# groupeLIAMG/ttcr

Measured on AMD Instinct MI355X. Metric: Mnodes/s per sweep-iteration (512^3 fp32 grid, first-order FSM), higher is better.
Workload: dtype f32

## Files before the change

### include/ttcr_amd.h

```cpp
#ifndef TTCR_AMD_H
#define TTCR_AMD_H

#include <stddef.h>
#include <stdint.h>

#ifdef __cplusplus
extern "C" {
#endif

typedef struct ttcr_fsm_grid ttcr_fsm_grid;

enum { TTCR_F32 = 0, TTCR_F64 = 1 };

enum {
    TTCR_OK = 0,
    TTCR_ERR_VALUE = 1,
    TTCR_ERR_RUNTIME = 2,
    TTCR_ERR_DEVICE = 3,
    TTCR_ERR_UNSUPPORTED = 4
};

int ttcr_fsm_device_count(void);

const char* ttcr_fsm_last_error(void);
// ... 121 lines not shown
int ttcr_fsm_multi_l_size(const ttcr_fsm_grid* g, size_t* n_rows, size_t* nnz);
int ttcr_fsm_get_multi_l(const ttcr_fsm_grid* g, long long* row_off, long long* cell, void* v);

typedef struct {
    double sweep_ms;
    double total_ms;
    long long kernel_launches;
    long long node_updates;
    long long evaluated_updates;
    int iterations;
    int n_sources;
} ttcr_fsm_timing;
int ttcr_fsm_last_timing(const ttcr_fsm_grid* g, ttcr_fsm_timing* out);
int ttcr_fsm_stopping_stats(const ttcr_fsm_grid* g, long long* reference_sums, long long* reference_sums_missed, long long* rounds);
int ttcr_fsm_prefill_swaps(const ttcr_fsm_grid* g, long long* swaps);
int ttcr_fsm_reference_change(ttcr_fsm_grid* g, const void* times, const void* field, int parallel, void* out);
int ttcr_fsm_last_kernel(const ttcr_fsm_grid* g, char* buf, size_t n);
int ttcr_fsm_unit_order(int dim, int dtype, int stage, int by_time, uint32_t nnx, uint32_t nny, uint32_t nnz, uint32_t* out,
                        size_t capacity, size_t* n_units);
const char* ttcr_fsm_build_id(void);

#ifdef __cplusplus
}
#endif
#endif
```

### ttcr_amd/_lib.py

```python
import ctypes as C
import os

HERE = os.path.dirname(os.path.abspath(__file__))
LIB_PATH = os.environ.get("TTCR_AMD_LIB") or os.path.join(HERE, "libttcr_amd.so")

TTCR_F32, TTCR_F64 = 0, 1
OK, ERR_VALUE, ERR_RUNTIME, ERR_DEVICE, ERR_UNSUPPORTED = 0, 1, 2, 3, 4

_P = C.c_void_p
_U32 = C.c_uint32
_D = C.c_double
_I = C.c_int


class Timing(C.Structure):
    _fields_ = [("sweep_ms", C.c_double), ("total_ms", C.c_double), ("kernel_launches", C.c_longlong),
                ("node_updates", C.c_longlong), ("evaluated_updates", C.c_longlong), ("iterations", C.c_int),
                ("n_sources", C.c_int)]


SYMBOLS = {
    "ttcr_fsm_device_count": (_I, []),
    "ttcr_fsm_last_error": (C.c_char_p, []),
    "ttcr_fsm3d_create": (_I, [C.POINTER(_P), _I, _I, _U32, _U32, _U32, _D, _D, _D, _D, _D, _I, _I, _I, _I, _I]),
# ... 14 lines not shown
    "ttcr_fsm_interp": (_I, [_P, _I, _I, _P, _P]),
    "ttcr_fsm_compute_slowness": (_I, [_P, _I, _P, _I, _P]),
    "ttcr_fsm_get_niter": (_I, [_P, _I, C.POINTER(_I), C.POINTER(_I)]),
    "ttcr_fsm_get_changes": (_I, [_P, _I, C.POINTER(_D), _I, C.POINTER(_D), _I]),
    "ttcr_fsm_get_reference_changes": (_I, [_P, _I, C.POINTER(_D), _I, C.POINTER(_D), _I]),
    "ttcr_fsm_n_slots": (_I, [_P]),
    "ttcr_fsm_n_nodes": (C.c_size_t, [_P]),
    "ttcr_fsm_n_cells": (C.c_size_t, [_P]),
    "ttcr_fsm_set_option": (_I, [_P, C.c_char_p, _D]),
    "ttcr_fsm_last_timing": (_I, [_P, C.POINTER(Timing)]),
    "ttcr_fsm_last_kernel": (_I, [_P, C.c_char_p, C.c_size_t]),
    "ttcr_fsm_build_id": (C.c_char_p, []),
    "ttcr_fsm_unit_order": (_I, [_I, _I, _I, _I, _U32, _U32, _U32, C.POINTER(_U32), C.c_size_t, C.POINTER(C.c_size_t)]),
    "ttcr_fsm_stopping_stats": (_I, [_P, C.POINTER(C.c_longlong), C.POINTER(C.c_longlong), C.POINTER(C.c_longlong)]),
    "ttcr_fsm_prefill_swaps": (_I, [_P, C.POINTER(C.c_longlong)]),
    "ttcr_fsm_reference_change": (_I, [_P, C.c_void_p, C.c_void_p, C.c_int, C.c_void_p]),
    "ttcr_fsm_rays_size": (_I, [_P, C.POINTER(C.c_size_t), C.POINTER(C.c_size_t)]),
    "ttcr_fsm_get_rays": (_I, [_P, _P, _P]),
    "ttcr_fsm_raytrace_rays": (_I, [_P, _I, _I, _P, _P, _I, _P, _P]),
    "ttcr_fsm_slot_rays_size": (_I, [_P, _I, C.POINTER(C.c_size_t), C.POINTER(C.c_size_t)]),
    "ttcr_fsm_get_slot_rays": (_I, [_P, _I, _P, _P]),
    "ttcr_fsm_raytrace_m": (_I, [_P, _I, _I, _P, _P, _I, _P, _P]),
    "ttcr_fsm_raytrace_rm": (_I, [_P, _I, _I, _P, _P, _I, _P, _P]),
    "ttcr_fsm_raytrace_multi_m": (_I, [_P, _I, _P, _P, _P, _P, _P, _P, _I]),
    "ttcr_fsm_multi_m_size": (_I, [_P, C.POINTER(C.c_size_t), C.POINTER(C.c_size_t)]),
    "ttcr_fsm_get_multi_m": (_I, [_P, _P, _P, _P]),
    "ttcr_fsm_raytrace_multi_tape": (_I, [_P, _I, _P, _P, _P, _P, _P, _P, C.POINTER(_P)]),
    "ttcr_fsm_tape_size": (_I, [_P, C.POINTER(C.c_size_t), C.POINTER(C.c_size_t), C.POINTER(C.c_size_t)]),
    "ttcr_fsm_tape_bytes": (_I, [_P, C.POINTER(C.c_size_t)]),
    "ttcr_fsm_tape_device": (_I, [_P, C.POINTER(_I)]),
# ... 89 lines not shown
```

### ttcr_amd/build.py

```python
import os
import shutil
import subprocess

HERE = os.path.dirname(os.path.abspath(__file__))
CSRC = os.path.join(HERE, "csrc")
OBJ = os.path.join(CSRC, "_obj")
LIB = os.path.join(HERE, "libttcr_amd.so")
INC = os.path.join("..", "..", "include", "ttcr_amd.h")
UNITS = {
    "fsm_capi.hip": ([], ["fsm_capi.hip", "fsm_kernels.h", "fsm_fast_api.h", "fsm_march_levels.inc", "fsm_fast.hip", "fsm_tape_api.h",
                          "fsm_tape.hip", "fsm_adjoint_api.h", "fsm_adjoint.hip", "fsm_unit_order.h", INC]),
    "fsm_fast.hip": ([], ["fsm_fast.hip", "fsm_fast_api.h", "fsm_kernels.h", "fsm_march_levels.inc"]),
    "fsm_tape.hip": ([], ["fsm_tape.hip", "fsm_tape_api.h"]),
    "fsm_adjoint.hip": ([], ["fsm_adjoint.hip", "fsm_adjoint_api.h", "fsm_kernels.h", "fsm_march_levels.inc"]),
}
SOURCES = list(UNITS)
DEPS = sorted({d for _, ds in UNITS.values() for d in ds})
FLAGS = ["--offload-arch=gfx950", "-O3", "-std=c++17", "-fPIC", "-ffp-contract=off",
         "-fno-fast-math", "-Wall", "-Wno-unused-result"]


def _hipcc():
    for c in (os.environ.get("HIPCC"), shutil.which("hipcc"), "/opt/rocm/bin/hipcc"):
        if c and os.path.exists(c):
            return c
    raise RuntimeError("hipcc not found")


def source_hash():
# ... 50 lines not shown
```

### ttcr_amd/csrc/fsm_capi.hip

```cpp
#include <hip/hip_runtime.h>

#include <algorithm>
#include <atomic>
#include <chrono>
#include <condition_variable>
#include <cmath>
#include <cstdio>
#include <cstdlib>
#include <cstring>
#include <limits>
#include <map>
#include <memory>
#include <mutex>
#include <sstream>
#include <stdexcept>
#include <string>
#include <thread>
#include <vector>

#include "../../include/ttcr_amd.h"
#include "fsm_kernels.h"
#include "fsm_fast_api.h"
#include "fsm_tape_api.h"
#include "fsm_adjoint_api.h"
// ... 117 lines not shown
    std::vector<int> niter, niterw;
    std::vector<int> phys;
    int P(int slot) const { return phys.empty() ? slot : phys[slot]; }
    int stopping_shortcuts = 3;
    int stopping_rule = 1;
    long long reference_sums = 0, reference_sums_missed = 0;
    long long refsum_rounds = 0;
    virtual void stopping_stats(long long* sums, long long* missed, long long* rounds) const {
        if (sums) *sums = reference_sums;
        if (missed) *missed = reference_sums_missed;
        if (rounds) *rounds = refsum_rounds;
    }
    virtual void reference_change_host(const void* times, const void* field, bool parallel, void* out) = 0;
    int pair_by_distance = 1;
    virtual void set_pair_layout(int) {}
    virtual long long prefill_swap_count() const { return 0; }
    int lone_chunk = 16;
    int arith = 0;
    int prefill = -1;
    std::vector<std::vector<double>> change_hist, change_histw;
    std::vector<std::vector<double>> ref_hist, ref_histw;
    virtual void get_reference_changes(int slot, double* first, int n_first, double* wen, int n_weno) const {
        if (slot < 0 || slot >= n_slots) throw ValueError("Thread number is larger than number of threads");
        slot = P(slot);
        for (int q = 0; q < n_first; ++q) first[q] = (!ref_hist.empty() && q < (int)ref_hist[slot].size()) ? ref_hist[slot][q] : std::nan("");
        for (int q = 0; q < n_weno; ++q) wen[q] = (!ref_histw.empty() && q < (int)ref_histw[slot].size()) ? ref_histw[slot][q] : std::nan("");
    }
    virtual void get_changes(int slot, double* first, int n_first, double* wen, int n_weno) const {
        if (slot < 0 || slot >= n_slots) throw ValueError("Thread number is larger than number of threads");
        slot = P(slot);
        for (int q = 0; q < n_first; ++q) first[q] = (!change_hist.empty() && q < (int)change_hist[slot].size()) ? change_hist[slot][q] : 0.0;
        for (int q = 0; q < n_weno; ++q) wen[q] = (!change_histw.empty() && q < (int)change_histw[slot].size()) ? change_histw[slot][q] : 0.0;
    }
    bool weno = false;
// ... 18 lines not shown
        else if (k == "mode") mode = (int)value;
        else if (k == "skip") skip = (int)value;
        else if (k == "tt_from_rp") ttrp = value != 0;
        else if (k == "interp_vel") interp_vel = value != 0;
        else if (k == "return_rays") return_rays = value != 0;
        else if (k == "pair_sources") pair_by_distance = value != 0;
        else if (k == "pair_layout") {
            if (value != -1 && value != 0 && value != 1) throw ValueError("option 'pair_layout': -1 (default), 0 or 1");
            set_pair_layout((int)value);
        }
        else if (k == "stopping_rule") stopping_rule = (int)value;
        else if (k == "stopping_shortcuts") { if (value < 0 || value > 3 || value != (double)(int)value) throw ValueError("option stopping_shortcuts: 0 ... 3"); stopping_shortcuts = (int)value; }
        else if (k == "prefill") {
            if (value != -1 && value != 0 && value != 1) throw ValueError("option 'prefill': -1 (default), 0 or 1");
            prefill = (int)value;
        } else if (k == "lone_chunk") {
            if (value != 8 && value != 16) throw ValueError("option 'lone_chunk': 8 or 16");
            lone_chunk = (int)value;
        }
        else if (k == "arith") {
            if (value != 0 && value != 1 && value != 2)
                throw ValueError("option 'arith': 0 (the reference's arithmetic), 1 (tolerance-grade fp32 where it stays within 1e-5 s RMS) or 2 (the WENO stage as well)");
            arith = (int)value;
        }
        else if (k == "walk_records") {
            if (value != 0 && !(value >= 1 && value <= (double)walk_step_limit && value == (double)(long)value))
                throw ValueError("option 'walk_records': 0 (default) or a whole number from 1 to the step limit of a walk");
            walk_records = (long)value;
        }
        else throw ValueError("unknown option '" + k + "'");
// ... 31 lines not shown
    T dx, dz, xmin, ymin, zmin, xmax, ymax, zmax, ox = 0, oy = 0, oz = 0;
    T epsilon;
    int nitermax;
    bool cell, translate;
    bool have_slowness = false;

    hipStream_t stream = nullptr;
    hipEvent_t ev0 = nullptr, ev1 = nullptr;
    DevBuf<T> d_s, d_cells, d_tt, d_rx, d_out;
    DevBuf<T> d_tt_alt;
    bool alt_filled = false;
    hipStream_t fill_stream = nullptr;
    hipEvent_t ev_fill = nullptr;
    long long prefill_swaps = 0;
    long long prefill_swap_count() const override { return prefill_swaps; }
    void set_pair_layout(int v) override { pair_layout = v; }
    DevBuf<int> d_rslot;
    DevBuf<RaySrc> d_rdesc;
    int weno_ch4_min = 8;
    int weno_c16_below = 3;
    int f64_c16_below = 5;
    int pre_min = 2;
    size_t xs_lds_bytes = 40000;
    int xs_lds_below = 2;
    size_t xs_dyn_lds(int batch) const { return (dim == 3 && stage == 0 && batch < xs_lds_below) ? xs_lds_bytes : 0; }
    int time_order_below = 1 << 30;
    DevBuf<T> d_gather;
    DevBuf<T> d_rsrc, d_rt0;
    DevBuf<int> d_rstat;
    DevBuf<T> d_ssh;
// ... 81 lines not shown
        }
        HIP_CHECK(hipStreamCreateWithFlags(&stream, hipStreamNonBlocking));
        HIP_CHECK(hipEventCreate(&ev0));
        HIP_CHECK(hipEventCreate(&ev1));
        d_s.reserve(n_nodes, 64);
        {
            long long pair_units_min = 6144;
            if (const char* e = std::getenv("TTCR_FSM_PAIR_UNITS")) pair_units_min = std::atoll(e);
            const long long patches = dim == 3 ? (long long)((ny + 1 + TileCfg<T, 3>::PJ - 1) / TileCfg<T, 3>::PJ) * ((nz + 1 + TileCfg<T, 3>::PK - 1) / TileCfg<T, 3>::PK) : 0;
            NS = (n_slots >= 2 && dim == 3 && !weno && (long long)n_slots * patches > pair_units_min) ? 2 : 1;
            ns_window = NS == 2 && (long long)n_slots * patches <= (5 * pair_units_min) / 2;
        }
        if (const char* e = std::getenv("TTCR_FSM_PAIR")) { NS = (std::atoi(e) != 0 && n_slots >= 2) ? 2 : 1; ns_window = false; }
        if (const char* e = std::getenv("TTCR_FSM_LAYOUT_LO")) layout_lo = std::atof(e);
        if (const char* e = std::getenv("TTCR_FSM_LAYOUT_HI")) layout_hi = std::atof(e);
        d_tt.reserve(n_nodes * (size_t)(n_slots + (n_slots & 1)), 64);
        mask_words = (n_nodes + 31) / 32;
        d_mask.reserve(mask_words * (size_t)n_slots);
        d_bbox.reserve(6 * (size_t)n_slots);
        d_slots.reserve(n_slots);
        d_lmask.reserve(n_slots);
        HIP_CHECK(hipHostMalloc((void**)&h_lmask, sizeof(int) * n_slots));
        d_change.reserve(n_slots);
        if (std::getenv("TTCR_FSM_PROF")) {
            prof_words = 8 + 4 * (size_t)(1 << 20);
            d_prof.reserve(prof_words);
            HIP_CHECK(hipMemset(d_prof.p, 0, prof_words * sizeof(unsigned long long)));
        }
        HIP_CHECK(hipHostMalloc((void**)&h_change, sizeof(double) * n_slots));
        HIP_CHECK(hipHostMalloc((void**)&h_slots, sizeof(int) * n_slots));
        HIP_CHECK(hipHostMalloc((void**)&h_abort, sizeof(int)));
        *h_abort = 0;
        HIP_CHECK(hipHostMalloc((void**)&h_iter, 2 * sizeof(int)));
        HIP_CHECK(hipHostMalloc((void**)&h_evals, sizeof(unsigned long long) * n_slots));
        HIP_CHECK(hipMemsetAsync(d_tt.p, 0, n_nodes * (size_t)(n_slots + (n_slots & 1)) * sizeof(T), stream));

        if (dim == 3) {
            using C = TileCfg<T, 3>;
            geom.NF = nx + 1; geom.NJ = ny + 1; geom.NK = nz + 1;
            geom.npj = (geom.NJ + C::PJ - 1) / C::PJ;
            geom.npk = (geom.NK + C::PK - 1) / C::PK;
            n_launch = count_launches(C::BL);
        } else {
            using C = TileCfg<T, 2>;
            geom.NF = nz + 1; geom.NJ = nx + 1; geom.NK = 1;
            geom.npj = (geom.NJ + C::PJ - 1) / C::PJ;
            geom.npk = 1;
            n_launch = count_launches(C::BL);
        }
        geom.n_nodes = (uint32_t)n_nodes;
// ... 113 lines not shown
        pa.sync = d_sync.p;
        pa.n_patches = n_patches;
        pa.batch = batch;
        pa.timeout_ticks = 300000000ull;
        pa.stamp = d_stamp.p;
        pa.iter_ptr = d_iter.p;
        pa.evals = d_evals.p;
        pa.nbf = nbf; pa.nbj = nbj; pa.nbk = nbk;
        pa.ndir = DIM == 3 ? 8 : 4;
        pa.skip = skip_now(batch) ? (std::getenv("TTCR_FSM_SKIP_ALL_DIRTY") ? 2 : 1) : 0;
        pa.cmap = d_cmap.p;
        pa.cw = cmap_words;
        pa.sw = std::getenv("TTCR_FSM_NO_SW") ? nullptr : d_sw.p;
        pa.n_sw_groups = n_groups();
        pa.n_sw_sweeps = sw_sweeps;

        const size_t wg_cap = (fsm_looped(DIM == 3, H) && persist_wgs > 0) ? (size_t)persist_wgs : ~(size_t)0;
        const dim3 block(C::PJ * C::PK), grid((unsigned)std::min<size_t>((size_t)n_patches * batch, wg_cap));
        const int ndir = DIM == 3 ? 8 : 4;
        {
            const bool pre_ = mode == 2 && !NO_PRE && (DIM == 2 || batch >= pre_min || dyn_lds > 0);
            char nm[160];
            std::snprintf(nm, sizeof nm, "fsm_sweep_persistent<%s,%d,%d,%d,%s,%s,%d,%d,%s,%s>", sizeof(T) == 4 ? "float" : "double", C::PJ, C::PK, CH,
                          DIM == 3 ? "true" : "false", skip_now(batch) ? "true" : "false", H, NSV, mode == 2 ? "true" : "false", pre_ ? "true" : "false");
            last_kernel = nm;
        }
        if (mode == 2) {
            pa.ssh = d_ssh.p;
            pa.ssh_stride = ssh_stride;
            pa.dir = 0;
            a.rf = a.rj = a.rk = a.rev = 0;
            a.s_sheared = nullptr;
            pa.timeout_ticks = 1000000000ull;
            const dim3 gridx((unsigned)std::min<size_t>((size_t)n_patches * batch * ndir, wg_cap));
            pa.order = d_order_xs[H == 2 ? 1 : 0][batch < time_order_below ? 1 : 0].p;
            const bool pre = DIM == 2 || batch >= pre_min || dyn_lds > 0;
            if constexpr (std::is_same<T, float>::value) {
                if (fast_now<H>() && (H == 1 || NSV == 1)) {
                    const FastCfg fc{H, DIM, NSV, CH, skip_now(batch), NO_PRE ? false : pre};
                    last_kernel.insert(last_kernel.size() - 1, ",1");
                    const hipError_t e = fsm_fast_launch(pa, fc, gridx.x, dyn_lds, stream);
                    if (e == hipErrorInvalidValue) throw std::logic_error("arith = 1: no such kernel (" + last_kernel + ")");
                    HIP_CHECK(e);
                    return;
                }
            }
            if constexpr (NO_PRE) {
                (void)pre;
                if (skip_now(batch))
                    fsm_sweep_persistent<T, C::PJ, C::PK, CH, DIM == 3, true, H, NSV, true><<<gridx, block, dyn_lds, stream>>>(pa);
                else
// ... 305 lines not shown
    bool ns_window = false;
    int pair_layout = -1;
    double last_eval_frac = -1;
    double layout_lo = 0.55, layout_hi = 0.70;
    void choose_layout() {
        if (!ns_window) return;
        int want = NS;
        if (pair_layout >= 0) want = pair_layout ? 2 : 1;
        else if (last_eval_frac >= 0) want = NS == 2 ? (last_eval_frac < layout_lo ? 1 : 2) : (last_eval_frac > layout_hi ? 2 : 1);
        if (want == NS) return;
        NS = want;
        graph_batches[0] = graph_batches[1] = -1;
        for (int q = 0; q < n_slots; ++q) phys[q] = q;
    }
    int n_groups() const { return (n_slots + NS - 1) / NS; }
    T* tt_ptr(int slot) const { return d_tt.p + (size_t)(slot / NS) * n_nodes * NS + slot % NS; }
    template <int H>
    bool fast_now() const { return sizeof(T) == 4 && (arith == 2 || (arith == 1 && !weno)); }
    bool prefill_on() const {
        if (prefill >= 0) return prefill != 0;
        const size_t bytes = n_nodes * (size_t)(n_slots + (n_slots & 1)) * sizeof(T);
        if (bytes < ((size_t)64 << 20)) return false;
        size_t free_b = 0, total_b = 0;
        if (hipMemGetInfo(&free_b, &total_b) != hipSuccess) return false;
        return d_tt_alt.p || (2 * bytes <= total_b / 2 && bytes + ((size_t)1 << 30) <= free_b);
    }

    int stage = 0;
    int skip_units_min = 2048;
    int skip_probe_min = 1024;
    bool probe_skip = true;
    int probe_off_calls = 0;
    int persist_wgs = 2048;
    bool in_probe_window(int entries) const {
        const long long u = (long long)n_patches * entries;
        return dim == 3 && sizeof(T) == 4 && u >= skip_probe_min && u < skip_units_min;
    }
    int skip_default(int entries) const {
        if (dim != 3) return 1;
        if (stage == 1) return 1;
// ... 384 lines not shown
        size_t tot_pts = 0;
        for (int b = 0; b < nb; ++b) tot_pts += tx_off[src_ids[b] + 1] - tx_off[src_ids[b]];
        std::vector<InitPoint<T>> pts;
        pts.reserve(tot_pts);
        std::vector<size_t> first(nb);
        for (int b = 0; b < nb; ++b) {
            first[b] = pts.size();
            for (int n = tx_off[src_ids[b]]; n < tx_off[src_ids[b] + 1]; ++n) pts.push_back(locate(tx + (size_t)nc * n, t0[n]));
        }
        d_pts.reserve(std::max<size_t>(tot_pts, 1));
        HIP_CHECK(hipMemcpyAsync(d_pts.p, pts.data(), pts.size() * sizeof(InitPoint<T>), hipMemcpyHostToDevice, stream));
        for (int b = 0; b < nb; ++b)
            HIP_CHECK(hipMemsetAsync(d_stamp.p + (size_t)(slot_ids[b] / NS) * n_bricks, 0xFF, n_bricks * sizeof(int), stream));
        std::vector<char> group_filled(n_groups(), 0);
        const bool all_slots = nb == n_slots && prefill_on();
        if (all_slots && alt_filled) {
            HIP_CHECK(hipStreamWaitEvent(stream, ev_fill, 0));
            std::swap(d_tt.p, d_tt_alt.p);
            std::swap(d_tt.n, d_tt_alt.n);
            std::swap(d_tt.guard, d_tt_alt.guard);
            alt_filled = false;
            ++prefill_swaps;
            graph_batches[0] = graph_batches[1] = -1;
            std::fill(group_filled.begin(), group_filled.end(), 1);
        }
        if (NS > 1) {
            std::vector<int> cnt(n_groups(), 0);
            for (int b = 0; b < nb; ++b) cnt[slot_ids[b] / NS] += 1;
            for (int gi = 0; gi < n_groups(); ++gi) {
                if (cnt[gi] != NS || group_filled[gi]) continue;
// ... 82 lines not shown
                } else {
                    n_entries = nb;
                    for (int b = 0; b < nb; ++b) { h_slots[b] = b < (int)active.size() ? active[b] : -1; h_lmask[b] = 1; }
                }
                HIP_CHECK(hipMemcpyAsync(d_slots.p, h_slots, sizeof(int) * n_entries, hipMemcpyHostToDevice, stream));
                HIP_CHECK(hipMemcpyAsync(d_lmask.p, h_lmask, sizeof(int) * n_entries, hipMemcpyHostToDevice, stream));
                HIP_CHECK(hipMemsetAsync(d_change.p, 0, sizeof(double) * n_slots, stream));
                iter_T = it_total;
                snapshots_before_iteration(active, it + 1);
                if (host_prof) { HIP_CHECK(hipStreamSynchronize(stream)); hp_mark("snapshots"); }
                stamps_ok = (it == 0 ? true : stamps_ok) && stamps_live_for(n_entries);
                h_iter[0] = it_total;
                h_iter[1] = (int)launch_epoch;
                launch_epoch += (persistent_now() && mode == 2) ? 1u : (unsigned)ndir;
                HIP_CHECK(hipMemcpyAsync(d_iter.p, h_iter, 2 * sizeof(int), hipMemcpyHostToDevice, stream));
                run_iteration(n_entries);
                HIP_CHECK(hipMemcpyAsync(h_change, d_change.p, sizeof(double) * n_slots, hipMemcpyDeviceToHost, stream));
                if (persistent_now()) HIP_CHECK(hipMemcpyAsync(h_abort, d_sync.p + 4, sizeof(int), hipMemcpyDeviceToHost, stream));
                HIP_CHECK(hipStreamSynchronize(stream));
                hp_mark("sweep-iteration");
                if (persistent_now() && *h_abort) {
                    HIP_CHECK(hipMemsetAsync(d_sync.p + 4, 0, sizeof(int), stream));
                    stage = 0;
                    throw DeviceError("persistent sweep kernel: a patch timed out waiting for its upwind neighbour");
                }
                ++it;
                ++it_total;
                std::vector<int> next;
                if (fixed_iters > 0) ref_change_last.assign(n_slots, std::nan(""));
                const std::vector<char> go = fixed_iters > 0 ? std::vector<char>(active.size(), 1) : decide_go_on(active, it);
                hp_mark("stopping rule");
                for (size_t q = 0; q < active.size(); ++q) {
                    const int s2 = active[q];
                    (stage == 0 ? niter : niterw)[s2] = it;
                    (stage == 0 ? change_hist : change_histw)[s2].push_back(h_change[s2]);
                    (stage == 0 ? ref_hist : ref_histw)[s2].push_back((int)ref_change_last.size() == n_slots ? ref_change_last[s2] : std::nan(""));
                    timing.node_updates += (long long)n_nodes * ndir;
                    prev2_change[s2] = prev_change[s2];
                    prev_change[s2] = h_change[s2];
                    if (go[q]) next.push_back(s2);
// ... 6 lines not shown
                for (int s2 : slot_ids)
                    HIP_CHECK(hipMemsetD32Async((hipDeviceptr_t)(d_stamp.p + (size_t)(s2 / NS) * n_bricks), it_total * (dim == 3 ? 8 : 4),
                                                n_bricks, stream));
            }
        }
        if (std::getenv("TTCR_FSM_DEBUG_SW")) {
            std::vector<unsigned long long> h((size_t)std::min(sw_sweeps, 40) * n_groups());
            HIP_CHECK(hipMemcpy(h.data(), d_sw.p, h.size() * sizeof(unsigned long long), hipMemcpyDeviceToHost));
            for (size_t q = 0; q < h.size(); ++q) std::fprintf(stderr, "%s%u/%u", q % n_groups() == 0 ? "\n[sw] " : " ", (unsigned)h[q], (unsigned)(h[q] >> 32));
            std::fprintf(stderr, "\n");
        }
        const bool was_persistent = mode >= 1 || weno;
        stage = 0;
        sync_clean = true;
        HIP_CHECK(hipEventRecord(ev1, stream));
        if (all_slots) {
            const size_t n_el = n_nodes * (size_t)(n_slots + (n_slots & 1));
            if (!fill_stream) {
                int lo = 0, hi = 0;
                HIP_CHECK(hipDeviceGetStreamPriorityRange(&lo, &hi));
                HIP_CHECK(hipStreamCreateWithPriority(&fill_stream, hipStreamNonBlocking, lo));
                HIP_CHECK(hipEventCreateWithFlags(&ev_fill, hipEventDisableTiming));
            }
            bool have_alt = true;
            try {
                d_tt_alt.reserve(n_el, 64);
            } catch (const DeviceError&) {
                (void)hipGetLastError();
                have_alt = false;
                prefill = 0;
            }
            if (have_alt) {
// ... 1070 lines not shown
        for (auto& r : rep) r->apply_option(k, value);
    }
    void set_slowness(const void* s, size_t n, bool on_device, bool c_order = false) override {
        for (auto& r : rep) r->set_slowness(s, n, on_device, c_order);
    }
    void get_slowness(void* out, size_t n) override { rep[0]->get_slowness(out, n); }
    void validate_points(int n_tx, const void* tx, int n_rx, const void* rx) override { rep[0]->validate_points(n_tx, tx, n_rx, rx); }
    void get_tt(int slot, void* out, size_t n) override { int l; GridBase& g = of(slot, l); g.get_tt(l, out, n); }
    void* tt_device(int slot) override { int l; GridBase& g = of(slot, l); return g.tt_device(l); }
    void* tt_device_view(int slot, size_t* stride) override { int l; GridBase& g = of(slot, l); return g.tt_device_view(l, stride); }
    void interp(int slot, int n, const void* pts, void* out) override { int l; GridBase& g = of(slot, l); g.interp(l, n, pts, out); }
    void compute_slowness(int n, const void* pts, bool translated, void* out) override { rep[0]->compute_slowness(n, pts, translated, out); }
    void get_niter(int slot, int* it, int* itw) const override { int l; GridBase& g = of(slot, l); g.get_niter(l, it, itw); }
    std::string kernel_name() const override { return rep[0]->kernel_name(); }
    long long prefill_swap_count() const override { long long a = 0; for (const auto& r : rep) a += r->prefill_swap_count(); return a; }
    void stopping_stats(long long* sums, long long* missed, long long* rounds) const override {
        long long a = 0, b = 0, c = 0;
        for (const auto& r : rep) { long long x = 0, y = 0, z = 0; r->stopping_stats(&x, &y, &z); a += x; b += y; c += z; }
        if (sums) *sums = a;
        if (missed) *missed = b;
        if (rounds) *rounds = c;
    }
    void reference_change_host(const void* times, const void* field, bool parallel, void* out) override { rep[0]->reference_change_host(times, field, parallel, out); }
    void get_changes(int slot, double* first, int n_first, double* wen, int n_weno) const override {
        int l; GridBase& g = of(slot, l); g.get_changes(l, first, n_first, wen, n_weno);
    }
    void get_reference_changes(int slot, double* first, int n_first, double* wen, int n_weno) const override {
        int l; GridBase& g = of(slot, l); g.get_reference_changes(l, first, n_first, wen, n_weno);
    }
    void rays_size(size_t* n_rays, size_t* n_points) const override { *n_rays = rays_off.size() - 1; *n_points = (size_t)rays_off.back(); }
// ... 1247 lines not shown
        out->total_ms = t.total_ms;
        out->kernel_launches = t.launches;
        out->node_updates = t.node_updates;
        out->evaluated_updates = t.evaluated_updates;
        out->iterations = t.iterations;
        out->n_sources = t.n_sources;
    });
}

int ttcr_fsm_stopping_stats(const ttcr_fsm_grid* g, long long* reference_sums, long long* reference_sums_missed, long long* rounds) {
    return guarded_on(g, [&] { g->impl->stopping_stats(reference_sums, reference_sums_missed, rounds); });
}
int ttcr_fsm_prefill_swaps(const ttcr_fsm_grid* g, long long* swaps) {
    return guarded_on(g, [&] { if (swaps) *swaps = g->impl->prefill_swap_count(); });
}
int ttcr_fsm_reference_change(ttcr_fsm_grid* g, const void* times, const void* field, int parallel, void* out) {
    return guarded_on(g, [&] {
        if (!times || !field || !out) throw ValueError("ttcr_fsm_reference_change: null argument");
        g->impl->reference_change_host(times, field, parallel != 0, out);
    });
}

int ttcr_fsm_last_kernel(const ttcr_fsm_grid* g, char* buf, size_t n) {
    return guarded_on(g, [&] {
        if (!buf || n == 0) throw ValueError("ttcr_fsm_last_kernel: no buffer");
        const std::string k = g->impl->kernel_name();
        std::snprintf(buf, n, "%s", k.c_str());
    });
}

// ... 16 lines not shown
        } else {
            PJ = dim == 3 ? TileCfg<double, 3>::PJ : TileCfg<double, 2>::PJ; PK = dim == 3 ? TileCfg<double, 3>::PK : 1;
            C = dim == 3 ? ChunkCfg<double, 3>::C : ChunkCfg<double, 2>::C;
        }
        const uint64_t npj = ((uint64_t)NJ + PJ - 1) / PJ, npk = ((uint64_t)NK + PK - 1) / PK;
        if (NF >= (1u << 30) || npj >= (1u << 14) || npk >= (1u << 14)) throw ValueError("grid too large for the patch index of the sweep kernel");
        *n_units = (size_t)(npj * npk) * (dim == 3 ? 8 : 4);
        if (!out) return;
        if (capacity < *n_units) throw ValueError("output buffer too small for the units of the launch");
        const std::vector<uint32_t> xs = fsm_xs_order(dim, (int)NF, (int)NJ, (int)NK, PJ, PK, C, stage == 0 ? 1 : 2, by_time != 0,
                                                      fsm_diag_order((int)npj, (int)npk));
        std::copy(xs.begin(), xs.end(), out);
    });
}

const char* ttcr_fsm_build_id(void) { return TTCR_BUILD_ID; }

}
```

### ttcr_amd/csrc/fsm_kernels.h

```cpp
#pragma once
#include <hip/hip_runtime.h>
#include <stdint.h>
#include <type_traits>

namespace ttcr_amd {

constexpr int FSM_BRICK = 16;

template <typename T> struct real_traits;
template <> struct real_traits<float> {
    static __host__ __device__ constexpr float max() { return 3.402823466e+38f; }
    static __device__ __forceinline__ float inf() { return __builtin_huge_valf(); }
};
template <> struct real_traits<double> {
    static __host__ __device__ constexpr double max() { return 1.7976931348623157e+308; }
    static __device__ __forceinline__ double inf() { return __builtin_huge_val(); }
};

__device__ __forceinline__ uint32_t idx_u32(double v) { return v < 0 ? 0u : (v >= 4294967295.0 ? 4294967295u : (uint32_t)v); }

__device__ __forceinline__ float rmin(float a, float b) { return a < b ? a : b; }
__device__ __forceinline__ double rmin(double a, double b) { return a < b ? a : b; }
__device__ __forceinline__ float rmax(float a, float b) { return a < b ? b : a; }
__device__ __forceinline__ double rmax(double a, double b) { return a < b ? b : a; }
// ... 404 lines not shown
    int* sync;
    int n_patches, batch;
    unsigned long long timeout_ticks;
    int* stamp;
    const int* iter_ptr;
    unsigned long long* evals;
    int nbf, nbj, nbk;
    int dir, ndir;
    int skip;
    unsigned long long* cmap;
    int cw;
    unsigned long long* sw;
    int n_sw_groups, n_sw_sweeps;
    const T* ssh;
    size_t ssh_stride;
};



__device__ __forceinline__ float ld_sc1(const float* p) {
    return __uint_as_float(__hip_atomic_load((const unsigned int*)p, __ATOMIC_RELAXED, __HIP_MEMORY_SCOPE_AGENT));
}
__device__ __forceinline__ double ld_sc1(const double* p) {
    return __longlong_as_double(__hip_atomic_load((const long long*)p, __ATOMIC_RELAXED, __HIP_MEMORY_SCOPE_AGENT));
}
__device__ __forceinline__ void st_sc1(float* p, float v) {
    __hip_atomic_store((unsigned int*)p, __float_as_uint(v), __ATOMIC_RELAXED, __HIP_MEMORY_SCOPE_AGENT);
}
__device__ __forceinline__ void st_sc1(double* p, double v) {
    __hip_atomic_store((long long*)p, __double_as_longlong(v), __ATOMIC_RELAXED, __HIP_MEMORY_SCOPE_AGENT);
// ... 409 lines not shown
        const int tka = IS3D ? ka2 / PK : 0, ntk = IS3D ? kb2 / PK - tka + 1 : 1;
        const int ia = lane & 3, ib = lane >> 2;
        if (ia >= ntj || ib >= ntk) return nullptr;
        return pa.sync + 8 + ((size_t)pd * pa.batch + z_) * pa.n_patches + ((tka + ib) * npj + tja + ia);
    };
    if constexpr (LOOPED) __syncthreads();
    if (tid == 0) {
        const int t_ = atomicAdd(pa.sync + (epoch & 3u), 1);
        if (t_ == 0) __hip_atomic_store(pa.sync + ((epoch + 2u) & 3u), 0, __ATOMIC_RELAXED, __HIP_MEMORY_SCOPE_AGENT);
        s_ticket = t_;
    }
    if (LOOPED && tid == 1) s_abort = __hip_atomic_load(pa.sync + 4, __ATOMIC_RELAXED, __HIP_MEMORY_SCOPE_AGENT);
    __syncthreads();
    if (LOOPED && s_abort) return false;
    const int ticket = __builtin_amdgcn_readfirstlane(s_ticket);
    const int oidx = ticket / pa.batch, z = ticket - oidx * pa.batch;
    if (oidx >= (XS ? pa.n_patches * pa.ndir : pa.n_patches)) return false;
    if (FSM_ENABLE_PROF == 1 && a.prof && ticket < 8192) prec = a.prof + 8 + 4 * 65536 + (size_t)ticket * 400;
    const uint32_t tile = pa.order[oidx];
    const int dir = XS ? (int)(tile >> 28) : pa.dir;
    const int TJ = XS ? (int)(tile & 0x3fffu) : (int)(tile & 0xffffu), TK = XS ? (int)((tile >> 14) & 0x3fffu) : (int)(tile >> 16);
    int* prog = pa.sync + 8 + ((size_t)(XS ? dir : 0) * pa.batch + z) * pa.n_patches;
    int* my_prog = prog + (TK * npj + TJ);
    int rf, rj, rk, rev;
    const T* __restrict__ Sg;
    if (XS) {
        int fam;
        if (IS3D) {
            rf = dir & 1; rj = (dir >> 1) & 1; rk = (dir >> 2) & 1;
            rev = rk;
// ... 2560 lines not shown
```

### ttcr_amd/rgrid.py

```python
import ctypes as C
import math

import numpy as np

from . import _lib

_verbose = 0


def set_verbose(v):
    global _verbose
    _verbose = int(v)


def _ptr(a):
    return a.ctypes.data_as(C.c_void_p)


def _row_groups(a):
    key = np.ascontiguousarray(a, dtype=np.float64) + 0.0
    n = key.shape[0]
    if n == 0:
        return np.zeros(0, dtype=np.intp), np.zeros(1, dtype=np.intp), key
    ne = key[1:] != key[:-1]
# ... 86 lines not shown
        return np.array(a[:n1]), np.array(b[:n2])

    def timing(self):
        t = _lib.Timing()
        _lib.check(self._lib.ttcr_fsm_last_timing(self._h, C.byref(t)))
        return {k: getattr(t, k) for k, _ in t._fields_}

    def stopping_stats(self):
        a, b, c = C.c_longlong(0), C.c_longlong(0), C.c_longlong(0)
        _lib.check(self._lib.ttcr_fsm_stopping_stats(self._h, C.byref(a), C.byref(b), C.byref(c)))
        return {"reference_sums": a.value, "reference_sums_missed": b.value, "rounds": c.value}

    def prefill_swaps(self):
        a = C.c_longlong(0)
        _lib.check(self._lib.ttcr_fsm_prefill_swaps(self._h, C.byref(a)))
        return a.value

    def reference_change(self, times, field, parallel=True):
        dt = self._dtype
        a = np.ascontiguousarray(times, dtype=dt).ravel()
        b = np.ascontiguousarray(field, dtype=dt).ravel()
        n = self.get_number_of_nodes()
        if a.size != n or b.size != n:
            raise ValueError('reference_change: fields of get_number_of_nodes() values expected')
        out = np.zeros(1, dtype=dt)
        _lib.check(self._lib.ttcr_fsm_reference_change(self._h, a.ctypes.data, b.ctypes.data, 1 if parallel else 0, out.ctypes.data))
        return out[0]

    def last_kernel(self):
        buf = C.create_string_buffer(256)
# ... 1250 lines not shown
```

Baseline: 94390.

## Fuse alternate travel-time buffer prefill into first sweep iteration kernel

Instead of filling the alternate travel-time buffer with max values on a separate low-priority stream after the solve, each sweep work-group writes a vectorized slice of that buffer at the start of its ticket during the first iteration. The aim is to hide the prefill memory traffic inside the sweep launch and avoid a separate fill pass competing for bandwidth. It also trims the tt allocation to omit the odd-slot padding when pairing is off. The cost is extra stores and register pressure in the sweep kernel prologue on every ticket of that iteration, plus a per-ticket branch checked in all launches.

```diff
diff --git a/include/ttcr_amd.h b/include/ttcr_amd.h
--- a/include/ttcr_amd.h
+++ b/include/ttcr_amd.h
@@ -159,10 +159,12 @@
 int ttcr_fsm_last_timing(const ttcr_fsm_grid* g, ttcr_fsm_timing* out);
 int ttcr_fsm_stopping_stats(const ttcr_fsm_grid* g, long long* reference_sums, long long* reference_sums_missed, long long* rounds);
 int ttcr_fsm_prefill_swaps(const ttcr_fsm_grid* g, long long* swaps);
+int ttcr_fsm_prefill_inline_fills(const ttcr_fsm_grid* g, long long* fills);
 int ttcr_fsm_reference_change(ttcr_fsm_grid* g, const void* times, const void* field, int parallel, void* out);
 int ttcr_fsm_last_kernel(const ttcr_fsm_grid* g, char* buf, size_t n);
 int ttcr_fsm_unit_order(int dim, int dtype, int stage, int by_time, uint32_t nnx, uint32_t nny, uint32_t nnz, uint32_t* out,
                         size_t capacity, size_t* n_units);
+int ttcr_fsm_prefill_slice(int dtype, uint64_t n_el, uint32_t n_tickets, uint32_t ticket, uint64_t* slice_len, uint64_t* begin, uint64_t* end);
 const char* ttcr_fsm_build_id(void);
 
 #ifdef __cplusplus
diff --git a/ttcr_amd/_lib.py b/ttcr_amd/_lib.py
--- a/ttcr_amd/_lib.py
+++ b/ttcr_amd/_lib.py
@@ -52,6 +52,8 @@
     "ttcr_fsm_unit_order": (_I, [_I, _I, _I, _I, _U32, _U32, _U32, C.POINTER(_U32), C.c_size_t, C.POINTER(C.c_size_t)]),
     "ttcr_fsm_stopping_stats": (_I, [_P, C.POINTER(C.c_longlong), C.POINTER(C.c_longlong), C.POINTER(C.c_longlong)]),
     "ttcr_fsm_prefill_swaps": (_I, [_P, C.POINTER(C.c_longlong)]),
+    "ttcr_fsm_prefill_inline_fills": (_I, [_P, C.POINTER(C.c_longlong)]),
+    "ttcr_fsm_prefill_slice": (_I, [_I, C.c_uint64, _U32, _U32, C.POINTER(C.c_uint64), C.POINTER(C.c_uint64), C.POINTER(C.c_uint64)]),
     "ttcr_fsm_reference_change": (_I, [_P, C.c_void_p, C.c_void_p, C.c_int, C.c_void_p]),
     "ttcr_fsm_rays_size": (_I, [_P, C.POINTER(C.c_size_t), C.POINTER(C.c_size_t)]),
     "ttcr_fsm_get_rays": (_I, [_P, _P, _P]),
diff --git a/ttcr_amd/build.py b/ttcr_amd/build.py
--- a/ttcr_amd/build.py
+++ b/ttcr_amd/build.py
@@ -9,10 +9,10 @@
 INC = os.path.join("..", "..", "include", "ttcr_amd.h")
 UNITS = {
     "fsm_capi.hip": ([], ["fsm_capi.hip", "fsm_kernels.h", "fsm_fast_api.h", "fsm_march_levels.inc", "fsm_fast.hip", "fsm_tape_api.h",
-                          "fsm_tape.hip", "fsm_adjoint_api.h", "fsm_adjoint.hip", "fsm_unit_order.h", INC]),
-    "fsm_fast.hip": ([], ["fsm_fast.hip", "fsm_fast_api.h", "fsm_kernels.h", "fsm_march_levels.inc"]),
+                          "fsm_tape.hip", "fsm_adjoint_api.h", "fsm_adjoint.hip", "fsm_unit_order.h", "fsm_prefill_slices.h", INC]),
+    "fsm_fast.hip": ([], ["fsm_fast.hip", "fsm_fast_api.h", "fsm_kernels.h", "fsm_march_levels.inc", "fsm_prefill_slices.h"]),
     "fsm_tape.hip": ([], ["fsm_tape.hip", "fsm_tape_api.h"]),
-    "fsm_adjoint.hip": ([], ["fsm_adjoint.hip", "fsm_adjoint_api.h", "fsm_kernels.h", "fsm_march_levels.inc"]),
+    "fsm_adjoint.hip": ([], ["fsm_adjoint.hip", "fsm_adjoint_api.h", "fsm_kernels.h", "fsm_march_levels.inc", "fsm_prefill_slices.h"]),
 }
 SOURCES = list(UNITS)
 DEPS = sorted({d for _, ds in UNITS.values() for d in ds})
diff --git a/ttcr_amd/csrc/fsm_capi.hip b/ttcr_amd/csrc/fsm_capi.hip
--- a/ttcr_amd/csrc/fsm_capi.hip
+++ b/ttcr_amd/csrc/fsm_capi.hip
@@ -155,10 +155,12 @@
     virtual void reference_change_host(const void* times, const void* field, bool parallel, void* out) = 0;
     int pair_by_distance = 1;
     virtual void set_pair_layout(int) {}
+    virtual long long prefill_inline_count() const { return 0; }
     virtual long long prefill_swap_count() const { return 0; }
     int lone_chunk = 16;
     int arith = 0;
     int prefill = -1;
+    int prefill_inline = -1;
     std::vector<std::vector<double>> change_hist, change_histw;
     std::vector<std::vector<double>> ref_hist, ref_histw;
     virtual void get_reference_changes(int slot, double* first, int n_first, double* wen, int n_weno) const {
@@ -207,6 +209,9 @@
         else if (k == "prefill") {
             if (value != -1 && value != 0 && value != 1) throw ValueError("option 'prefill': -1 (default), 0 or 1");
             prefill = (int)value;
+        } else if (k == "prefill_inline") {
+            if (value != -1 && value != 0 && value != 1) throw ValueError("option 'prefill_inline': -1 (default), 0 or 1");
+            prefill_inline = (int)value;
         } else if (k == "lone_chunk") {
             if (value != 8 && value != 16) throw ValueError("option 'lone_chunk': 8 or 16");
             lone_chunk = (int)value;
@@ -268,6 +273,8 @@
     hipEvent_t ev_fill = nullptr;
     long long prefill_swaps = 0;
     long long prefill_swap_count() const override { return prefill_swaps; }
+    long long prefill_inline_fills = 0;
+    long long prefill_inline_count() const override { return prefill_inline_fills; }
     void set_pair_layout(int v) override { pair_layout = v; }
     DevBuf<int> d_rslot;
     DevBuf<RaySrc> d_rdesc;
@@ -379,7 +386,7 @@
         if (const char* e = std::getenv("TTCR_FSM_PAIR")) { NS = (std::atoi(e) != 0 && n_slots >= 2) ? 2 : 1; ns_window = false; }
         if (const char* e = std::getenv("TTCR_FSM_LAYOUT_LO")) layout_lo = std::atof(e);
         if (const char* e = std::getenv("TTCR_FSM_LAYOUT_HI")) layout_hi = std::atof(e);
-        d_tt.reserve(n_nodes * (size_t)(n_slots + (n_slots & 1)), 64);
+        d_tt.reserve(n_nodes * tt_fields(), 64);
         mask_words = (n_nodes + 31) / 32;
         d_mask.reserve(mask_words * (size_t)n_slots);
         d_bbox.reserve(6 * (size_t)n_slots);
@@ -398,7 +405,7 @@
         *h_abort = 0;
         HIP_CHECK(hipHostMalloc((void**)&h_iter, 2 * sizeof(int)));
         HIP_CHECK(hipHostMalloc((void**)&h_evals, sizeof(unsigned long long) * n_slots));
-        HIP_CHECK(hipMemsetAsync(d_tt.p, 0, n_nodes * (size_t)(n_slots + (n_slots & 1)) * sizeof(T), stream));
+        HIP_CHECK(hipMemsetAsync(d_tt.p, 0, n_nodes * tt_fields() * sizeof(T), stream));
 
         if (dim == 3) {
             using C = TileCfg<T, 3>;
@@ -542,6 +549,9 @@
         pa.sw = std::getenv("TTCR_FSM_NO_SW") ? nullptr : d_sw.p;
         pa.n_sw_groups = n_groups();
         pa.n_sw_sweeps = sw_sweeps;
+        pa.fill_dst = nullptr;
+        pa.fill_slice = 0;
+        pa.fill_n = 0;
 
         const size_t wg_cap = (fsm_looped(DIM == 3, H) && persist_wgs > 0) ? (size_t)persist_wgs : ~(size_t)0;
         const dim3 block(C::PJ * C::PK), grid((unsigned)std::min<size_t>((size_t)n_patches * batch, wg_cap));
@@ -563,6 +573,13 @@
             const dim3 gridx((unsigned)std::min<size_t>((size_t)n_patches * batch * ndir, wg_cap));
             pa.order = d_order_xs[H == 2 ? 1 : 0][batch < time_order_below ? 1 : 0].p;
             const bool pre = DIM == 2 || batch >= pre_min || dyn_lds > 0;
+            if (fill_arm) {
+                pa.fill_dst = d_tt_alt.p;
+                pa.fill_n = n_nodes * tt_fields();
+                pa.fill_slice = fsm_fill_slice_len(pa.fill_n, (size_t)n_patches * batch * ndir, 16 / sizeof(T));
+                fill_arm = false;
+                fill_in_flight = true;
+            }
             if constexpr (std::is_same<T, float>::value) {
                 if (fast_now<H>() && (H == 1 || NSV == 1)) {
                     const FastCfg fc{H, DIM, NSV, CH, skip_now(batch), NO_PRE ? false : pre};
@@ -898,16 +915,25 @@
         for (int q = 0; q < n_slots; ++q) phys[q] = q;
     }
     int n_groups() const { return (n_slots + NS - 1) / NS; }
+    size_t tt_fields() const { return (size_t)n_slots + ((ns_window || NS == 2) ? (size_t)(n_slots & 1) : 0); }
     T* tt_ptr(int slot) const { return d_tt.p + (size_t)(slot / NS) * n_nodes * NS + slot % NS; }
     template <int H>
     bool fast_now() const { return sizeof(T) == 4 && (arith == 2 || (arith == 1 && !weno)); }
     bool prefill_on() const {
         if (prefill >= 0) return prefill != 0;
-        const size_t bytes = n_nodes * (size_t)(n_slots + (n_slots & 1)) * sizeof(T);
+        const size_t bytes = n_nodes * tt_fields() * sizeof(T);
         if (bytes < ((size_t)64 << 20)) return false;
         size_t free_b = 0, total_b = 0;
         if (hipMemGetInfo(&free_b, &total_b) != hipSuccess) return false;
         return d_tt_alt.p || (2 * bytes <= total_b / 2 && bytes + ((size_t)1 << 30) <= free_b);
+    }
+    bool fill_arm = false;
+    bool fill_in_flight = false;
+    bool inline_fill_now(int entries) const {
+        if (prefill_inline == 0 || !d_tt_alt.p || d_tt_alt.n < n_nodes * tt_fields()) return false;
+        if (mode != 2 || stage != 0 || use_graph >= 2) return false;
+        if (prefill_inline == 1) return true;
+        return dim == 3 && !fast_now<1>() && (long long)n_patches * entries >= skip_units_min;
     }
 
     int stage = 0;
@@ -1322,6 +1348,8 @@
             HIP_CHECK(hipMemsetAsync(d_stamp.p + (size_t)(slot_ids[b] / NS) * n_bricks, 0xFF, n_bricks * sizeof(int), stream));
         std::vector<char> group_filled(n_groups(), 0);
         const bool all_slots = nb == n_slots && prefill_on();
+        fill_arm = fill_in_flight = false;
+        bool inline_filled = false;
         if (all_slots && alt_filled) {
             HIP_CHECK(hipStreamWaitEvent(stream, ev_fill, 0));
             std::swap(d_tt.p, d_tt_alt.p);
@@ -1434,7 +1462,9 @@
                 h_iter[1] = (int)launch_epoch;
                 launch_epoch += (persistent_now() && mode == 2) ? 1u : (unsigned)ndir;
                 HIP_CHECK(hipMemcpyAsync(d_iter.p, h_iter, 2 * sizeof(int), hipMemcpyHostToDevice, stream));
+                fill_arm = it_total == 0 && all_slots && !alt_filled && inline_fill_now(n_entries);
                 run_iteration(n_entries);
+                fill_arm = false;
                 HIP_CHECK(hipMemcpyAsync(h_change, d_change.p, sizeof(double) * n_slots, hipMemcpyDeviceToHost, stream));
                 if (persistent_now()) HIP_CHECK(hipMemcpyAsync(h_abort, d_sync.p + 4, sizeof(int), hipMemcpyDeviceToHost, stream));
                 HIP_CHECK(hipStreamSynchronize(stream));
@@ -1444,6 +1474,7 @@
                     stage = 0;
                     throw DeviceError("persistent sweep kernel: a patch timed out waiting for its upwind neighbour");
                 }
+                if (fill_in_flight) { inline_filled = true; fill_in_flight = false; }
                 ++it;
                 ++it_total;
                 std::vector<int> next;
@@ -1480,8 +1511,11 @@
         stage = 0;
         sync_clean = true;
         HIP_CHECK(hipEventRecord(ev1, stream));
-        if (all_slots) {
-            const size_t n_el = n_nodes * (size_t)(n_slots + (n_slots & 1));
+        if (all_slots && inline_filled) {
+            alt_filled = true;
+            ++prefill_inline_fills;
+        } else if (all_slots) {
+            const size_t n_el = n_nodes * tt_fields();
             if (!fill_stream) {
                 int lo = 0, hi = 0;
                 HIP_CHECK(hipDeviceGetStreamPriorityRange(&lo, &hi));
@@ -2582,6 +2616,7 @@
     void get_niter(int slot, int* it, int* itw) const override { int l; GridBase& g = of(slot, l); g.get_niter(l, it, itw); }
     std::string kernel_name() const override { return rep[0]->kernel_name(); }
     long long prefill_swap_count() const override { long long a = 0; for (const auto& r : rep) a += r->prefill_swap_count(); return a; }
+    long long prefill_inline_count() const override { long long a = 0; for (const auto& r : rep) a += r->prefill_inline_count(); return a; }
     void stopping_stats(long long* sums, long long* missed, long long* rounds) const override {
         long long a = 0, b = 0, c = 0;
         for (const auto& r : rep) { long long x = 0, y = 0, z = 0; r->stopping_stats(&x, &y, &z); a += x; b += y; c += z; }
@@ -3859,6 +3894,9 @@
 int ttcr_fsm_prefill_swaps(const ttcr_fsm_grid* g, long long* swaps) {
     return guarded_on(g, [&] { if (swaps) *swaps = g->impl->prefill_swap_count(); });
 }
+int ttcr_fsm_prefill_inline_fills(const ttcr_fsm_grid* g, long long* fills) {
+    return guarded_on(g, [&] { if (fills) *fills = g->impl->prefill_inline_count(); });
+}
 int ttcr_fsm_reference_change(ttcr_fsm_grid* g, const void* times, const void* field, int parallel, void* out) {
     return guarded_on(g, [&] {
         if (!times || !field || !out) throw ValueError("ttcr_fsm_reference_change: null argument");
@@ -3905,6 +3943,19 @@
     });
 }
 
+int ttcr_fsm_prefill_slice(int dtype, uint64_t n_el, uint32_t n_tickets, uint32_t ticket, uint64_t* slice_len, uint64_t* begin, uint64_t* end) {
+    return guarded([&] {
+        if (dtype != TTCR_F32 && dtype != TTCR_F64) throw ValueError("dtype must be TTCR_F32 or TTCR_F64");
+        if (n_tickets == 0) throw ValueError("a launch has at least one ticket");
+        const size_t slice = fsm_fill_slice_len((size_t)n_el, n_tickets, dtype == TTCR_F32 ? 4 : 2);
+        size_t b = 0, e = 0;
+        fsm_fill_slice_range((size_t)n_el, slice, ticket, &b, &e);
+        if (slice_len) *slice_len = slice;
+        if (begin) *begin = b;
+        if (end) *end = e;
+    });
+}
+
 const char* ttcr_fsm_build_id(void) { return TTCR_BUILD_ID; }
 
 }
diff --git a/ttcr_amd/csrc/fsm_kernels.h b/ttcr_amd/csrc/fsm_kernels.h
--- a/ttcr_amd/csrc/fsm_kernels.h
+++ b/ttcr_amd/csrc/fsm_kernels.h
@@ -2,6 +2,8 @@
 #include <hip/hip_runtime.h>
 #include <stdint.h>
 #include <type_traits>
+
+#include "fsm_prefill_slices.h"
 
 namespace ttcr_amd {
 
@@ -442,6 +444,9 @@
     int n_sw_groups, n_sw_sweeps;
     const T* ssh;
     size_t ssh_stride;
+    T* fill_dst;
+    size_t fill_slice;
+    size_t fill_n;
 };
 
 
@@ -881,6 +886,21 @@
     __syncthreads();
     if (LOOPED && s_abort) return false;
     const int ticket = __builtin_amdgcn_readfirstlane(s_ticket);
+    if (pa.fill_slice) {
+        constexpr int VE = 16 / (int)sizeof(T);
+        typedef T FillV __attribute__((ext_vector_type(VE)));
+        size_t fb, fe;
+        fsm_fill_slice_range(pa.fill_n, pa.fill_slice, (size_t)(unsigned)ticket, &fb, &fe);
+        T* __restrict__ fdst = pa.fill_dst;
+        T fmax = real_traits<T>::max();
+        asm volatile("" : "+v"(fmax));
+        FillV fv;
+#pragma unroll
+        for (int q = 0; q < VE; ++q) fv[q] = fmax;
+        for (size_t i = fb + (size_t)tid * VE; i + VE <= fe; i += (size_t)NT * VE) *reinterpret_cast<FillV*>(fdst + i) = fv;
+        const size_t rem = (fe - fb) % VE;
+        if ((size_t)tid < rem) fdst[fe - rem + tid] = fmax;
+    }
     const int oidx = ticket / pa.batch, z = ticket - oidx * pa.batch;
     if (oidx >= (XS ? pa.n_patches * pa.ndir : pa.n_patches)) return false;
     if (FSM_ENABLE_PROF == 1 && a.prof && ticket < 8192) prec = a.prof + 8 + 4 * 65536 + (size_t)ticket * 400;
diff --git a/ttcr_amd/csrc/fsm_prefill_slices.h b/ttcr_amd/csrc/fsm_prefill_slices.h
--- /dev/null
+++ b/ttcr_amd/csrc/fsm_prefill_slices.h
@@ -0,0 +1,24 @@
+#pragma once
+#include <cstddef>
+
+#if defined(__HIPCC__) || defined(__CUDACC__)
+#define FSM_SLICE_HD __host__ __device__
+#else
+#define FSM_SLICE_HD
+#endif
+
+FSM_SLICE_HD inline size_t fsm_fill_slice_len(size_t n_el, size_t n_tickets, size_t vec) {
+    if (n_tickets == 0) n_tickets = 1;
+    const size_t per = (n_el + n_tickets - 1) / n_tickets;
+    const size_t len = (per + vec - 1) / vec * vec;
+    return len ? len : vec;
+}
+
+FSM_SLICE_HD inline void fsm_fill_slice_range(size_t n_el, size_t slice, size_t ticket, size_t* b, size_t* e) {
+    size_t lo;
+    if (__builtin_mul_overflow(ticket, slice, &lo)) lo = n_el;
+    const size_t b_ = lo < n_el ? lo : n_el;
+    const size_t e_ = n_el - b_ < slice ? n_el : b_ + slice;
+    *b = b_;
+    *e = e_;
+}
diff --git a/ttcr_amd/rgrid.py b/ttcr_amd/rgrid.py
--- a/ttcr_amd/rgrid.py
+++ b/ttcr_amd/rgrid.py
@@ -124,6 +124,11 @@
     def prefill_swaps(self):
         a = C.c_longlong(0)
         _lib.check(self._lib.ttcr_fsm_prefill_swaps(self._h, C.byref(a)))
+        return a.value
+
+    def prefill_inline_fills(self):
+        a = C.c_longlong(0)
+        _lib.check(self._lib.ttcr_fsm_prefill_inline_fills(self._h, C.byref(a)))
         return a.value
 
     def reference_change(self, times, field, parallel=True):
```

Result: faster. 95770 (median of 6 runs) (+1.5%).
